# open-speech/HTK

Hardware: AMD Instinct MI355X
Metric: herest_gmm_frame_state_loglik_per_sec (higher is better)
Workload: dtype f32 (scores: bf16x3 split operands, fp32 accumulate) + f64 (alpha / beta with fp32-transcendental log-add, accumulators); 1 GPU; HERest EM iteration (pass + accumulator all-reduce + model update), 5000 tied states x 16 mix, D=39, 1250 x 500-frame utterances per GPU (BASELINE config[2]: 10k utterances sharded 8-way); states=5000, mix=16, utts_per_gpu=1250, frames=500, chunks=1, update=HERest -m 3 -v 0.01, on the device

## Files before the change

### htk_amd/csrc/comm.hip

```cpp
#include <hip/hip_runtime.h>
#include <dlfcn.h>
#include <cstdlib>
#include <cstring>
#include <algorithm>
#include "internal.h"
#include "hipcheck.h"

typedef struct { char internal[128]; } rcclId;
typedef void *rcclComm;
typedef int (*fnGetUniqueId)(rcclId *);
typedef int (*fnCommInitRank)(rcclComm *, int, rcclId, int);
typedef int (*fnAllReduce)(const void *, void *, size_t, int, int, rcclComm, hipStream_t);
typedef int (*fnCommDestroy)(rcclComm);
typedef const char *(*fnGetErrorString)(int);

static struct { void *h; fnGetUniqueId getId; fnCommInitRank init; fnAllReduce allReduce; fnCommDestroy destroy; fnGetErrorString err; } g_rccl;

static int rccl_bind()
{
   if (g_rccl.h) return HTKAMD_OK;
   const char *names[] = {"librccl.so.1", "librccl.so", "/opt/rocm/lib/librccl.so.1", nullptr};
   void *h = nullptr;
   for (int i = 0; names[i] && !h; i++) h = dlopen(names[i], RTLD_NOW | RTLD_GLOBAL);
   if (!h) { htkamd_set_error("comm: RCCL not found (librccl.so.1): %s", dlerror()); return HTKAMD_ENODEV; }
// ... 57 lines not shown
}

__global__ void k_wire_pack(const double *__restrict__ v, float *__restrict__ w, size_t n)
{
   for (size_t i = (size_t)blockIdx.x * blockDim.x + threadIdx.x; i < n; i += (size_t)gridDim.x * blockDim.x) w[i] = (float)v[i];
}
__global__ void k_wire_unpack(const float *__restrict__ w, double *__restrict__ v, size_t n)
{
   for (size_t i = (size_t)blockIdx.x * blockDim.x + threadIdx.x; i < n; i += (size_t)gridDim.x * blockDim.x) v[i] = (double)w[i];
}

extern "C" int htkamd_accs_wire_round(htkamd_accs *a, void *stream)
{
   if (!a) { htkamd_set_error("accs_wire_round: NULL argument"); return HTKAMD_EINVAL; }
   const size_t bulk = a->lay.nEgs;
   float *w = nullptr;
   HIPCHECK(hipMalloc(&w, sizeof(float) * bulk));
   k_wire_pack<<<1024, 256, 0, (hipStream_t)stream>>>(a->d_vec, w, bulk);
   HIPCHECK(hipGetLastError());
   k_wire_unpack<<<1024, 256, 0, (hipStream_t)stream>>>(w, a->d_vec, bulk);
   HIPCHECK(hipGetLastError());
   HIPCHECK(hipStreamSynchronize((hipStream_t)stream));
   HIPCHECK(hipFree(w));
   return HTKAMD_OK;
}

extern "C" int htkamd_accs_allreduce_wire(htkamd_accs *a, htkamd_comm *c, int wire, void *stream)
{
   if (wire == HTKAMD_WIRE_F64) return htkamd_accs_allreduce(a, c, stream);
   if (!a || !c || wire != HTKAMD_WIRE_F32) { htkamd_set_error("accs_allreduce_wire: bad argument"); return HTKAMD_EINVAL; }
   if (c->nRanks == 1) return HTKAMD_OK;
   const size_t bulk = a->lay.nEgs, tail = a->lay.total - bulk;
   if (c->wireCap < bulk) {
      if (c->d_wire) HIPCHECK(hipFree(c->d_wire));
      c->d_wire = nullptr; c->wireCap = 0;
      HIPCHECK(hipMalloc(&c->d_wire, sizeof(float) * bulk));
      c->wireCap = bulk;
   }
   hipStream_t st = (hipStream_t)stream;
   k_wire_pack<<<1024, 256, 0, st>>>(a->d_vec, c->d_wire, bulk);
   HIPCHECK(hipGetLastError());
   RCCLCHECK(g_rccl.allReduce(c->d_wire, c->d_wire, bulk, 7 , 0 , c->c, st));
   RCCLCHECK(g_rccl.allReduce(a->d_vec + bulk, a->d_vec + bulk, tail, 8 , 0, c->c, st));
   k_wire_unpack<<<1024, 256, 0, st>>>(c->d_wire, a->d_vec, bulk);
   HIPCHECK(hipGetLastError());
   return HTKAMD_OK;
}

extern "C" int htkamd_accs_state_ranges(htkamd_accs *a, int state0, int state1, int withRest, size_t off[7], size_t len[7], int *n)
{
   if (!a || !off || !len || !n) { htkamd_set_error("accs_state_ranges: NULL argument"); return HTKAMD_EINVAL; }
   const htkamd_model *m = a->m;
   if (state0 < 0 || state1 > m->S || state0 > state1) { htkamd_set_error("accs_state_ranges: states [%d, %d) outside the set's %d", state0, state1, m->S); return HTKAMD_EINVAL; }
   if (a->stateOrder == 0) {
      a->stateOrder = (m->G == m->C && m->NSt <= 1 && !m->tiedMix) ? 1 : -1;
      for (int c = 0; c < m->C && a->stateOrder == 1; c++) if (m->h_compGauss[c] != c) a->stateOrder = -1;
   }
   if (a->stateOrder < 0) { htkamd_set_error("accs_state_ranges: the set's components do not own their Gaussians in state order (shared pdfs, several streams or tied mixtures): exchange the vector whole"); return HTKAMD_EMODEL; }
   const size_t g0 = (size_t)m->h_stateCompOff[state0], g1 = (size_t)m->h_stateCompOff[state1], D = (size_t)m->D;
   int k = 0;
   auto put = [&](size_t o, size_t l) { if (l) { off[k] = o; len[k] = l; k++; } };
   put(a->lay.mu + g0 * D, (g1 - g0) * D); put(a->lay.muOcc + g0, g1 - g0);
   put(a->lay.va + g0 * D, (g1 - g0) * D); put(a->lay.vaOcc + g0, g1 - g0);
   put(a->lay.wt + g0, g1 - g0); put(a->lay.wtOcc + (size_t)state0, (size_t)(state1 - state0));
   if (withRest) put(a->lay.tr, a->lay.nEgs - a->lay.tr);
   *n = k;
   return HTKAMD_OK;
}

struct RangeSet { size_t off[7], len[7], start[8]; int n; };
template <typename W, bool PACK>
__global__ void k_ranges(double *__restrict__ v, W *__restrict__ w, RangeSet r)
{
   const size_t total = r.start[r.n];
   for (size_t i = (size_t)blockIdx.x * blockDim.x + threadIdx.x; i < total; i += (size_t)gridDim.x * blockDim.x) {
      int k = 0;
      while (k + 1 < r.n && i >= r.start[k + 1]) k++;
      const size_t j = r.off[k] + (i - r.start[k]);
      if (PACK) w[i] = (W)v[j]; else v[j] = (double)w[i];
   }
}

static int ranges_launch(htkamd_accs *a, int n, const size_t *off, const size_t *len, int wire, void *buf, hipStream_t st, bool pack, size_t *totalOut)
{
   if (!a || n < 0 || n > 7 || (n && (!off || !len)) || (wire != HTKAMD_WIRE_F32 && wire != HTKAMD_WIRE_F64)) { htkamd_set_error("accs ranges: bad argument"); return HTKAMD_EINVAL; }
   RangeSet r; r.n = n; r.start[0] = 0;
   for (int k = 0; k < n; k++) {
      if (off[k] + len[k] > a->lay.total) { htkamd_set_error("accs ranges: range %d beyond the vector", k); return HTKAMD_EINVAL; }
      r.off[k] = off[k]; r.len[k] = len[k]; r.start[k + 1] = r.start[k] + len[k];
   }
   if (totalOut) *totalOut = r.start[n];
   if (r.start[n] == 0) return HTKAMD_OK;
   if (!buf) { htkamd_set_error("accs ranges: NULL buffer"); return HTKAMD_EINVAL; }
   const unsigned blocks = (unsigned)std::min<size_t>((r.start[n] + 255) / 256, 2048);
   if (wire == HTKAMD_WIRE_F32) { if (pack) k_ranges<float, true><<<blocks, 256, 0, st>>>(a->d_vec, (float *)buf, r); else k_ranges<float, false><<<blocks, 256, 0, st>>>(a->d_vec, (float *)buf, r); }
   else { if (pack) k_ranges<double, true><<<blocks, 256, 0, st>>>(a->d_vec, (double *)buf, r); else k_ranges<double, false><<<blocks, 256, 0, st>>>(a->d_vec, (double *)buf, r); }
   HIPCHECK(hipGetLastError());
   return HTKAMD_OK;
}

extern "C" int htkamd_accs_pack_ranges(htkamd_accs *a, int n, const size_t *off, const size_t *len, int wire, void *dst, void *stream)
{
   return ranges_launch(a, n, off, len, wire, dst, (hipStream_t)stream, true, nullptr);
}

extern "C" int htkamd_accs_unpack_ranges(htkamd_accs *a, int n, const size_t *off, const size_t *len, int wire, const void *src, void *stream)
{
   return ranges_launch(a, n, off, len, wire, (void *)src, (hipStream_t)stream, false, nullptr);
}

extern "C" int htkamd_accs_allreduce_states(htkamd_accs *a, htkamd_comm *c, int wire, int state0, int state1, int withRest, void *stream)
// ... 42 lines not shown
```

### htk_amd/csrc/fb.hip

```cpp
#include <hip/hip_runtime.h>
#include <cstdio>
#include <cstdlib>
#include <cstring>
#include <cmath>
#include <algorithm>
#include <vector>
#include <thread>
#include <mutex>
#include <condition_variable>
#include <functional>
#include "internal.h"
#include "hipcheck.h"
#include "kernels.h"
#include "devbuf.h"

static constexpr char fbOwner[] = "fb";
typedef DevBufT<fbOwner> DevBuf;

struct PrepPool {
   std::vector<std::thread> th;
   std::mutex mu;
   std::condition_variable cvGo, cvDone;
   std::function<void(int)> job;
   int generation = 0, pending = 0, nJobs = 0;
// ... 83 lines not shown
   {
      for_each([](auto &v, int) { v.clear(); });
      outp = beta = gam = 0; frameStates = 0; nCellsMax = QMax = TMax = 1; nThrMax = 64; rc = HTKAMD_OK; err[0] = 0;
   }
};

struct UttClasses {
   static constexpr int N = 13;
   struct Range { int first, n; };
   static int index(int family, int W) { return W == 0 ? 4 : (family ? 4 * family + 1 : 0) + (W == 1 ? 0 : W == 2 ? 1 : W == 4 ? 2 : 3); }
   void set(const std::vector<int> (&cls)[N], std::vector<int> &list)
   {
      list.clear();
      for (int c = 0; c < N; c++) { list.insert(list.end(), cls[c].begin(), cls[c].end()); off[c + 1] = (int)list.size(); }
   }
   Range of(int family, int W) const { const int c = index(family, W); return {off[c], off[c + 1] - off[c]}; }
   Range general() const { return of(FB_LANE_PER_MODEL, 0); } int nGeneral() const { return general().n; }
   int nLr() const { return off[N] - of(FB_LEFT_TO_RIGHT, 1).first; }
   bool anyOffLr() const { return of(FB_LEFT_TO_RIGHT, 1).first > 0; }
private:
   int off[N + 1] = {};
};

struct ResLayout {
   size_t nUtt;
   size_t status() const { return sizeof(double) * nUtt; }
   size_t counter() const { return (sizeof(double) + sizeof(int)) * nUtt; }
   size_t flag() const { return counter() + sizeof(int); } size_t bytes() const { return counter() + 2 * sizeof(int); }
};

enum { UTT_NO_TEE = 1, UTT_ALL_LR = 2 };

struct htkamd_fb : BatchTables {
   htkamd_model *m = nullptr;
   int nUtt = 0;
   int debug = 0;
   int forceGeneral = 0;
   int noStatePath = 0;
   int noLrPath = 0;
   int topoVersion = 0;
   std::vector<unsigned char> uttFlags;
   UttClasses cls;
   size_t gamTotal = 0, betaWTotal = 0, alphaWTotal = 0;
   int totalFrames = 0, nCellsMax = 1, QMax = 1, TMax = 1, blockDim = 64;
   long long frameStates = 0;
   const float *dX = nullptr;
   DevBuf d_arena;
   DevBuf d_qLo, d_qHi, d_aLo, d_aHi, d_outp, d_beta, d_gam, d_alpha, d_pr;
   DevBuf d_betaW;
   DevBuf d_tmE, d_tmMaxP;
   DevBuf d_outpU;
   DevBuf d_alphaW, d_qBeam, d_aBeam, d_trPart, d_hits, d_hitCtl;
   DevBuf d_sink;
   DevBuf d_stCnt, d_stBucket;
   DevBuf d_laneRec;
   bool mixStateLast = false;
   bool mixDeferred = false;
   FbArgs *faMix = nullptr;
   const int *qBeamLast = nullptr;
   DevBuf d_transOff, d_trOccOff, d_counter;
   DevBuf d_rec, d_recSorted, d_recCtl;
   int recCapForce = 0;
   PrepPool *pool = nullptr; std::vector<PrepChunk> *chunks = nullptr;
   void *h_arena = nullptr; size_t h_arenaCap = 0;
   void *h_res = nullptr; size_t h_resCap = 0;
   hipEvent_t evRes = nullptr; bool resPending = false;
   bool f16Pass = false;
   hipEvent_t ev[6] = {}, evK[2] = {}, evCopy = nullptr;
   hipStream_t resStream = nullptr;
   bool timed = false, copyPending = false, scored = false;
   int evMode = 0, evModeLast = 0;
   ResLayout res() const { return {(size_t)nUtt}; }
};

static bool compat_revisit(const htkamd_model *m) { return (m->compat & HTKAMD_COMPAT_STREAM_REVISIT) && m->NSt > 1 && m->NSt != 3 && !m->tiedMix; }

extern "C" int htkamd_fb_create(htkamd_model *m, htkamd_fb **out)
{
   if (!m || !out) { htkamd_set_error("fb_create: NULL argument"); return HTKAMD_EINVAL; }
   if (m->fullc) { htkamd_set_error("fb_create: forward-backward on FULLC models is not supported yet (its mixture statistics are diagonal)"); return HTKAMD_EMODEL; }
   if (m->maxM > 4096) { htkamd_set_error("fb_create: %d mixture components per state not supported", m->maxM); return HTKAMD_EMODEL; }
   htkamd_fb *fb = new htkamd_fb();
   fb->m = m;
   auto fail = [&](const char *what, hipError_t e) { htkamd_set_error("fb_create: %s: %s", what, hipGetErrorString(e)); htkamd_fb_destroy(fb); return HTKAMD_EHIP; };
   hipError_t e;
   for (hipEvent_t *v : {&fb->ev[0], &fb->ev[1], &fb->ev[2], &fb->ev[3], &fb->ev[4], &fb->ev[5], &fb->evK[0], &fb->evK[1]})
      if ((e = hipEventCreate(v)) != hipSuccess) return fail("hipEventCreate", e);
   if ((e = hipEventCreateWithFlags(&fb->evCopy, hipEventDisableTiming)) != hipSuccess) return fail("hipEventCreate", e);
   if ((e = hipStreamCreateWithFlags(&fb->resStream, hipStreamNonBlocking)) != hipSuccess) return fail("hipStreamCreate", e);
   int rc;
   if ((rc = fb->d_counter.reserve(64)) || (rc = fb->d_transOff.reserve(sizeof(int) * (m->nT + 1))) || (rc = fb->d_trOccOff.reserve(sizeof(int) * (m->nT + 1)))) { htkamd_fb_destroy(fb); return rc; }
   if ((e = hipMemcpy(fb->d_transOff.p, m->h_transOff, sizeof(int) * (m->nT + 1), hipMemcpyHostToDevice)) != hipSuccess ||
       (e = hipMemcpy(fb->d_trOccOff.p, m->h_trOccOff, sizeof(int) * (m->nT + 1), hipMemcpyHostToDevice)) != hipSuccess) return fail("hipMemcpy", e);
   *out = fb;
   return HTKAMD_OK;
}

extern "C" void htkamd_fb_destroy(htkamd_fb *fb)
{
   if (!fb) return;
   if (fb->h_arena) (void)hipHostFree(fb->h_arena);
   if (fb->h_res) (void)hipHostFree(fb->h_res);
   delete fb->pool; delete fb->chunks; delete fb->faMix;
   for (hipEvent_t v : fb->ev) if (v) (void)hipEventDestroy(v);
   for (hipEvent_t v : {fb->evCopy, fb->evRes, fb->evK[0], fb->evK[1]}) if (v) (void)hipEventDestroy(v);
   if (fb->resStream) (void)hipStreamDestroy(fb->resStream);
   delete fb;
// ... 415 lines not shown
   fa.stateCompOff = m->d_stateCompOff; fa.compGauss = m->d_compGauss;
   fa.NSt = m->NSt; fa.outpU = (const float *)fb->d_outpU.p; fa.dimStream = m->d_dimStream;
   fa.compatRevisit = compat_revisit(m) && !fb->nextSame.empty(); fa.nextSame = fb->nextSame.dev;
   fa.transOff = (const int *)fb->d_transOff.p; fa.trOccOff = (const int *)fb->d_trOccOff.p;
   fa.compLogWt = m->d_compLogWt; fa.gparam = m->d_gparam; fa.mean = m->d_mean; fa.laddTab = m->d_laddTab;
   fa.PS = m->PS; fa.D = m->D; fa.maxN = m->maxN; fa.maxM = m->maxM;
   fa.nCellsMax = fb->nCellsMax; fa.QMax = fb->QMax; fa.TMax = fb->TMax;
   fa.acc = accs->d_vec; fa.lay = accs->lay;
   fa.pruneInit = cfg->pruneInit; fa.pruneInc = cfg->pruneInc; fa.pruneLim = cfg->pruneLim;
   fa.minLogExp = m->minLogExp; fa.minFrwdP = cfg->minFrwdP; fa.uFlags = cfg->uFlags;
   fa.gamTotal = fb->gamTotal; fa.gamOffByUtt = fb->gamOff.dev; fa.gamChunkUtt = fb->gamChunkUtt.dev;
   return fa;
}

struct LdsSizes { size_t beta, alpha; };
static LdsSizes fb_lds_sizes(const FbArgs &fa)
{
   const size_t nc = fa.nCellsMax, qm = fa.QMax + 3, mn = fa.maxN, tm = (size_t)fa.TMax + 3;
   auto r8 = [](size_t x) { return (x + 7) & ~(size_t)7; };
   const size_t ldsTab = r8((size_t)LADD_NK * (LADD_DEG + 1) * 8);
   return {2 * r8(nc * 8) + r8(qm * 8) + r8(nc * mn * 4) + 4 * r8(qm * 4) + r8(32) + ldsTab,
           2 * r8(nc * 8) + r8(3 * nc * 8) + r8(qm * 8) + r8(nc * (mn + 1) * 8) + ldsTab + r8(3 * nc * 4) + 2 * r8(nc * mn * 4) + 4 * r8(qm * 4) + 2 * r8(tm * 2)};
}

static const int clsW[4] = {1, 2, 4, 8};

static int fb_reserve_lr(htkamd_fb *fb, const htkamd_fb_config *cfg, FbArgs &fa, bool fastLadd, hipStream_t s)
{
   const htkamd_model *m = fb->m;
   int rc;
   size_t rows = 0;
   for (int W : clsW) rows += (size_t)fb->cls.of(FB_LEFT_TO_RIGHT, W).n * htkamd_stats_lr_chunks(fb->TMax) * W;
   const size_t nfr = fb->totalFrames ? fb->totalFrames : 1;
   if ((rc = fb->d_laneRec.reserve(sizeof(LaneRec) * (fb->slotState.size() + 1))) || (rc = fb->d_sink.reserve(256))) return rc;
   fa.laneRec = (LaneRec *)fb->d_laneRec.p; fa.sink = (double *)fb->d_sink.p;
   if ((rc = fb->d_alphaW.reserve(sizeof(double) * (fb->alphaWTotal + 64))) || (rc = fb->d_qBeam.reserve(sizeof(int) * (nfr + 2))) ||
       (rc = fb->d_aBeam.reserve(sizeof(int) * (nfr + 2))) || (rc = fb->d_trPart.reserve(sizeof(double) * htkamd_stats_lr_row_doubles() * (rows + 256))) ||
       (rc = fb->d_hits.reserve(sizeof(MixHit) * (rows * htkamd_stats_lr_region_cap() + 64))) || (rc = fb->d_hitCtl.reserve(sizeof(int) * (rows + 1))))
      return rc;
   fa.alphaW = (double *)fb->d_alphaW.p; fa.qBeam = (int *)fb->d_qBeam.p; fa.aBeam = (int *)fb->d_aBeam.p; fa.trPart = (double *)fb->d_trPart.p;
   fa.hits = (MixHit *)fb->d_hits.p; fa.hitCtl = (int *)fb->d_hitCtl.p; fa.nHitRegions = (int)rows; fa.hitRegionCap = htkamd_stats_lr_region_cap();
   fa.hitSlots = (m->NSt > 1 || m->tiedMix) ? 1 : 0;
   fa.qBeamNP = fb->qBeamNP.dev;
   if (htkamd_beta_lr_is_lean(fa, fastLadd)) fa.qBeam = const_cast<int *>(fb->qBeamNP.dev);
   fb->qBeamLast = fa.qBeam;
   fb->mixStateLast = false;
   fa.fastMath = fastLadd ? 1 : 0;
   if (fb->recCapForce == 0 && !fa.hitSlots && m->maxM <= 16 && (m->D == 39 || m->D == 26 || m->D == 13) &&
       (cfg->uFlags & (HTKAMD_UPMEANS | HTKAMD_UPVARS | HTKAMD_UPMIXES))) {
      size_t cap = 64;
      while (cap < 65536 && cap * (size_t)m->S < (size_t)16 * fb->totalFrames) cap <<= 1;
      while (cap > 64 && cap * (size_t)m->S * sizeof(HitS) > ((size_t)1 << 30)) cap >>= 1;
      { const char *e = getenv("HTKAMD_ST_CAP"); if (e && atoi(e) > 0) cap = (size_t)atoi(e); }
      if ((rc = fb->d_stCnt.reserve(sizeof(int) * (3 * (size_t)m->S + 4))) || (rc = fb->d_stBucket.reserve(sizeof(HitS) * cap * (size_t)m->S))) return rc;
      fb->mixStateLast = true;
      fa.stCnt = (int *)fb->d_stCnt.p; fa.nTiedStates = m->S; fa.stBucket = (HitS *)fb->d_stBucket.p; fa.stCap = (int)cap;
      HIPCHECK(hipMemsetAsync(fa.stCnt, 0, sizeof(int) * (3 * (size_t)m->S + 4), s));
   }
   return HTKAMD_OK;
}

struct FamilyKernels { int family; int (*beta)(const FbArgs &, int, bool, hipStream_t); int (*alpha)(const FbArgs &, int, bool, hipStream_t); };
static const FamilyKernels familyKernels[] = {{FB_LANE_PER_MODEL, htkamd_launch_beta_w, htkamd_launch_alpha_w},
                                              {FB_LANE_PER_STATE, htkamd_launch_beta_s, htkamd_launch_alpha_s},
                                              {FB_LEFT_TO_RIGHT, htkamd_launch_beta_lr, htkamd_launch_alpha_lr}};

static int fb_recursions(htkamd_fb *fb, const FbArgs &fa, const LdsSizes &lds, bool fastLadd, bool noEv, hipStream_t s)
{
   int rc;
   for (int pass = 0; pass < 2; pass++) {
      FbArgs fc = fa;
      const UttClasses::Range g = fb->cls.general();
      fc.uttList = fb->uttList.dev + g.first; fc.nList = g.n;
      if (g.n > 0 && (rc = pass == 0 ? htkamd_launch_beta(fc, fb->blockDim, lds.beta, s) : htkamd_launch_alpha(fc, fb->blockDim, lds.alpha, s))) return rc;
      for (const FamilyKernels &k : familyKernels)
         for (int c = 3; c >= 0; c--) {
            const UttClasses::Range r = fb->cls.of(k.family, clsW[c]);
            fc.uttList = fb->uttList.dev + r.first; fc.nList = r.n;
            if ((rc = (pass == 0 ? k.beta : k.alpha)(fc, clsW[c], fastLadd, s))) return rc;
         }
      if (!noEv) HIPCHECK(hipEventRecord(fb->ev[2 + pass], s));
   }
   return HTKAMD_OK;
}

static int fb_stats_lr(htkamd_fb *fb, const FbArgs &fa, bool fastLadd, bool noEv, hipStream_t s)
{
   int rc;
   FbArgs fc = fa;
   size_t rowOff = 0;
   for (int c = 3; c >= 0; c--) {
      const UttClasses::Range r = fb->cls.of(FB_LEFT_TO_RIGHT, clsW[c]);
      fc.uttList = fb->uttList.dev + r.first; fc.nList = r.n;
      fc.trPart = fa.trPart ? fa.trPart + rowOff * htkamd_stats_lr_row_doubles() : nullptr;
      fc.hits = fa.hits ? fa.hits + rowOff * htkamd_stats_lr_region_cap() : nullptr; fc.hitCtl = fa.hitCtl ? fa.hitCtl + rowOff : nullptr;
      rowOff += (size_t)fc.nList * htkamd_stats_lr_chunks(fb->TMax) * clsW[c];
      if ((rc = htkamd_launch_stats_lr(fc, clsW[c], fastLadd, s))) return rc;
   }
   if (!noEv) HIPCHECK(hipEventRecord(fb->ev[4], s));
   return HTKAMD_OK;
}

static int fb_mix_stats(htkamd_fb *fb, const htkamd_fb_config *cfg, FbArgs &fa, bool defer, hipStream_t s)
{
   const htkamd_model *m = fb->m;
   const int nLr = fb->cls.nLr();
   int rc;
   if (!(cfg->uFlags & (HTKAMD_UPMEANS | HTKAMD_UPVARS | HTKAMD_UPMIXES))) return HTKAMD_OK;
   if ((cfg->uFlags & (HTKAMD_UPMEANS | HTKAMD_UPVARS)) && fb->recCapForce >= 0) {
      const size_t cap = fb->recCapForce > 0 ? (size_t)fb->recCapForce : std::min<size_t>((size_t)16 * fb->totalFrames + 4096, (size_t)1 << 30);
// ... 297 lines not shown
```

### htk_amd/csrc/fb_kernels.hip

```cpp
#include <hip/hip_runtime.h>
#include <cstring>
#include <cstdlib>
#include "internal.h"
#include "hipcheck.h"
#include "kernels.h"
#include "ladd.h"

#define ladd(x, y, mle) ladd_tab((x), (y), (mle), ltab)

#define EXPFLOOR (-100.0)

struct CellMeta {
   int q, i, N, mc0, ms0;
};

struct LdsCarve {
   char *p;
   __device__ explicit LdsCarve(void *base) : p((char *)base) {}
   template <typename T> __device__ T *take(size_t n)
   {
      T *r = (T *)p;
      p += ((n * sizeof(T) + 7) & ~(size_t)7);
      return r;
   }
// ... 846 lines not shown
   const bool upMu = a.uFlags & HTKAMD_UPMEANS, upVa = a.uFlags & HTKAMD_UPVARS;
   const int nWaves = (gridDim.x * blockDim.x) >> 6;
   for (int g = (blockIdx.x * blockDim.x + threadIdx.x) >> 6; g < G; g += nWaves) {
      const int r0 = start[g], r1 = start[g + 1];
      if (r0 == r1) continue;
      for (int k0 = 0; k0 < D; k0 += 64) {
         const int k = k0 + lane;
         const float mean = (k < D) ? a.mean[(size_t)g * D + k] : 0.0f;
         double sMu = 0.0, sVa = 0.0, sL = 0.0;
         for (int rb = r0; rb < r1; rb += 64) {
            const int nb = (r1 - rb < 64) ? r1 - rb : 64;
            MixRec mine; mine.frame = 0; mine.L = 0.0;
            if (lane < nb) mine = a.recSorted[rb + lane];
            sL += mine.L;
            for (int i = 0; i < nb; i += 4) {
               float xv[4]; double Lv[4];
#pragma unroll
               for (int e = 0; e < 4; e++) {
                  const int ii = (i + e < nb) ? i + e : nb - 1;
                  const int fr = __shfl(mine.frame, ii);
                  Lv[e] = (i + e < nb) ? __shfl(mine.L, ii) : 0.0;
                  xv[e] = (k < D) ? a.X[(size_t)fr * D + k] : 0.0f;
               }
#pragma unroll
               for (int e = 0; e < 4; e++) {
                  if (i + e >= nb) break;
                  const float z = xv[e] - mean;
                  const double L = Lv[e];
                  if (upMu && upVa) {
                     const float zl = (float)((double)z * L);
                     sMu += (double)zl; sVa += (double)(z * zl);
                  } else if (upMu) sMu += (double)z * L;
                  else if (upVa) sVa += (double)(z * z) * L;
               }
            }
         }
         if (k < D) {
            if (upMu && sMu != 0.0) atomicAdd(a.acc + a.lay.mu + (size_t)g * D + k, sMu);
            if (upVa && sVa != 0.0) atomicAdd(a.acc + a.lay.va + (size_t)g * D + k, sVa);
         }
         if (k0 == 0) {
#pragma unroll
            for (int o = 32; o > 0; o >>= 1) sL += __shfl_xor(sL, o);
            if (lane == 0) {
               if (upMu) atomicAdd(a.acc + a.lay.muOcc + g, sL);
               if (upVa) atomicAdd(a.acc + a.lay.vaOcc + g, sL);
            }
         }
      }
   }
}

#define MS_EU 8
template <int DT, int MODE>
__global__ __launch_bounds__(64, MS_EU) void k_mixstate(FbArgs a)
{
#define MS_CHUNK 32
#define MS_CAP 128
#define MS_PARTS 4
   constexpr int GS = 16, HPS = 64 / GS, NQ = (DT + 1) / 2, XS = (DT + 3) & ~3;
   constexpr int CH = MS_CHUNK;
   __shared__ float xs[CH * XS];
   __shared__ double Lt[CH][GS];
   __shared__ double hSeed[CH];
   const int st = a.stBase + blockIdx.x, lane = threadIdx.x, grp = lane / GS, sub = lane % GS;
   const int nst = a.stCnt[st] < a.stCap ? a.stCnt[st] : a.stCap;
   const int part = blockIdx.y;
   const int r0 = part * MS_CAP, r1 = (part == (int)gridDim.y - 1 || r0 + MS_CAP > nst) ? nst : r0 + MS_CAP;
   if (r0 >= nst) return;
   const HitS *bucket = a.stBucket + (size_t)st * a.stCap;
   const int c0 = a.stateCompOff[st], M = a.stateCompOff[st + 1] - c0;
   const bool single = (M == 1 || a.maxM == 1);
   constexpr bool upMu = (MODE & 1) != 0, upVa = (MODE & 2) != 0;
   const bool upWt = a.uFlags & HTKAMD_UPMIXES;
   __shared__ float4 pl[NQ][GS];
   int g = 0;
   float wt = 0.0f, gcst = 0.0f;
   if (sub < M) {
      g = a.compGauss[c0 + sub];
      wt = a.compLogWt[c0 + sub];
      gcst = a.gparam[(size_t)g * a.PS + 2 * DT];
      if (grp == 0) {
         const float4 *P4 = (const float4 *)(a.gparam + (size_t)g * a.PS);
#pragma unroll
         for (int q = 0; q < NQ; q++) { const float4 pv = P4[q]; pl[q][sub] = make_float4(pv.x, pv.z, pv.y, pv.w); }
      }
   }
   float meanR[GS];
   const int gOfLane = (lane < M) ? a.compGauss[c0 + lane] : 0;
#pragma unroll
   for (int m = 0; m < GS; m++) { const int gm_ = __builtin_amdgcn_readlane(gOfLane, m); meanR[m] = (m < M && lane < DT) ? a.mean[(size_t)gm_ * DT + lane] : 0.0f; }
   double sMu[GS], sVa[GS];
#pragma unroll
   for (int m = 0; m < GS; m++) { sMu[m] = 0.0; sVa[m] = 0.0; }
   double wtAcc = 0.0;
   int nTriples = 0;
   const double minF = uniform_f64((double)a.minFrwdP);

   for (int base = r0; base < r1; base += CH) {
      const int n = (r1 - base < CH) ? r1 - base : CH;
      __syncthreads();
      int hfr = 0;
      if (lane < n) { const HitS h = bucket[base + lane]; hfr = h.frame; hSeed[lane] = h.seed; }
      for (int r = 0; r < n; r++) {
         const int fr = __builtin_amdgcn_readlane(hfr, r);
         if (lane < DT)
// ... 25 lines not shown
                  sum += tt[0];
                  if (2 * q + 1 < DT) sum += tt[1];
               }
               const float prob = -0.5f * sum;
               const double x = (seed + (double)wt) + (double)prob;
               if (-x < minF) { pass = true; Lr = a.fastMath ? (double)__builtin_amdgcn_exp2f((float)x * 1.44269504088896341f) : exp(x); }
            }
         }
         if (have) Lt[h][sub] = pass ? Lr : 0.0;
         wtAcc += pass ? Lr : 0.0;
         nTriples += pass ? 1 : 0;
      }
      __syncthreads();
      if (upMu || upVa) {
         unsigned long long bmAll[GS];
#pragma unroll
         for (int m4 = 0; m4 < GS; m4 += 4) {
            double Lq[4];
#pragma unroll
            for (int i = 0; i < 4; i++) Lq[i] = (lane < n) ? Lt[lane][m4 + i] : 0.0;
#pragma unroll
            for (int i = 0; i < 4; i++) bmAll[m4 + i] = __ballot(Lq[i] != 0.0);
         }
#pragma unroll
         for (int m = 0; m < GS; m++) {
            if (m < M) {
               unsigned long long bm = bmAll[m];
               double mu = sMu[m], va = sVa[m];
               const float mean = meanR[m];
               while (bm) {
                  double Lv[4]; float xv[4];
#pragma unroll
                  for (int i = 0; i < 4; i++) {
                     const bool live = bm != 0;
                     const int h = live ? (int)__builtin_ctzll(bm) : 0;
                     bm &= bm - 1;
                     Lv[i] = live ? Lt[h][m] : 0.0;
                     xv[i] = xs[h * XS + (lane < DT ? lane : 0)];
                  }
#pragma unroll
                  for (int i = 0; i < 4; i++) {
                     const double L = Lv[i];
                     const float z = xv[i] - mean;
                     if constexpr (upMu && upVa) { const float zl = (float)((double)z * L); mu += (double)zl; va += (double)(z * zl); }
                     else if constexpr (upMu) mu += (double)z * L;
                     else va += (double)(z * z) * L;
                  }
               }
               sMu[m] = mu; sVa[m] = va;
            }
         }
      }
   }
#pragma unroll
   for (int m = 0; m < GS; m++) {
      if (m < M && lane < DT) {
         const int gm = a.compGauss[c0 + m];
         if (upMu && sMu[m] != 0.0) atomicAdd(a.acc + a.lay.mu + (size_t)gm * DT + lane, sMu[m]);
         if (upVa && sVa[m] != 0.0) atomicAdd(a.acc + a.lay.va + (size_t)gm * DT + lane, sVa[m]);
      }
   }
   double w = wtAcc;
   w += __shfl_xor(w, 16); w += __shfl_xor(w, 32);
   if (grp == 0 && sub < M && w != 0.0) {
      if (upWt) atomicAdd(a.acc + a.lay.wt + c0 + sub, w);
      if (upMu) atomicAdd(a.acc + a.lay.muOcc + g, w);
      if (upVa) atomicAdd(a.acc + a.lay.vaOcc + g, w);
   }
#pragma unroll
   for (int o = 32; o > 0; o >>= 1) nTriples += __shfl_xor(nTriples, o);
   if (lane == 0) { if (part == 0) a.stCnt[a.nTiedStates + 4 + 2 * st] = nst; atomicAdd(a.stCnt + a.nTiedStates + 5 + 2 * st, nTriples); }
   double so = (sub < M) ? w : 0.0;
#pragma unroll
   for (int o = GS / 2; o > 0; o >>= 1) so += __shfl_xor(so, o);
   if (lane == 0 && so != 0.0) atomicAdd(a.acc + a.lay.wtOcc + st, so);
}

bool htkamd_mixstate_applies(const FbArgs &a) { return a.stCnt && a.stBucket && !a.hitSlots && a.maxM <= 16 && (a.D == 39 || a.D == 26 || a.D == 13); }
int htkamd_launch_mixstate_range(const FbArgs &a_in, int st0, int st1, hipStream_t s)
{
   if (st0 < 0 || st1 > a_in.nTiedStates || st0 > st1) { htkamd_set_error("mixture statistics: state range [%d, %d) outside the set's %d", st0, st1, a_in.nTiedStates); return HTKAMD_EINVAL; }
   if (st0 == st1) return HTKAMD_OK;
   FbArgs a = a_in;
   a.stBase = st0;
   const int S = st1 - st0;
   const int mode = ((a.uFlags & HTKAMD_UPMEANS) ? 1 : 0) | ((a.uFlags & HTKAMD_UPVARS) ? 2 : 0);
#define MS_LAUNCH(DT_) \
   do { \
      if (mode == 3) hipLaunchKernelGGL((k_mixstate<DT_, 3>), dim3(S, MS_PARTS), dim3(64), 0, s, a); \
      else if (mode == 1) hipLaunchKernelGGL((k_mixstate<DT_, 1>), dim3(S, MS_PARTS), dim3(64), 0, s, a); \
      else if (mode == 2) hipLaunchKernelGGL((k_mixstate<DT_, 2>), dim3(S, MS_PARTS), dim3(64), 0, s, a); \
      else hipLaunchKernelGGL((k_mixstate<DT_, 0>), dim3(S, MS_PARTS), dim3(64), 0, s, a); \
   } while (0)
   if (a.D == 39) MS_LAUNCH(39); else if (a.D == 26) MS_LAUNCH(26); else MS_LAUNCH(13);
#undef MS_LAUNCH
   HIPCHECK(hipGetLastError());
   return HTKAMD_OK;
}

static int set_lds_limit(const void *fn, size_t lds)
{
   if (lds > 64 * 1024)
      HIPCHECK(hipFuncSetAttribute(fn, hipFuncAttributeMaxDynamicSharedMemorySize, (int)lds));
   return HTKAMD_OK;
}

int htkamd_launch_beta(const FbArgs &a, int blockDim, size_t lds, hipStream_t s)
{
   int rc = set_lds_limit((const void *)k_beta, lds);
   if (rc) return rc;
   hipLaunchKernelGGL(k_beta, dim3(a.nList), dim3(blockDim), lds, s, a);
   HIPCHECK(hipGetLastError());
   return HTKAMD_OK;
}

int htkamd_launch_alpha(const FbArgs &a, int blockDim, size_t lds, hipStream_t s)
{
   int rc = set_lds_limit((const void *)k_alpha, lds);
   if (rc) return rc;
   hipLaunchKernelGGL(k_alpha, dim3(a.nList), dim3(blockDim), lds, s, a);
   HIPCHECK(hipGetLastError());
   return HTKAMD_OK;
}

int htkamd_launch_mixstats(const FbArgs &a_in, hipStream_t s, bool dense, bool listed, bool deferState)
{
   if (!dense && !listed) return HTKAMD_OK;
   FbArgs a = a_in;
   dense = dense && a.gamTotal > 0;
   const bool stateOnly = listed && !dense && htkamd_mixstate_applies(a);
   if (stateOnly) a.rec = nullptr;
// ... 421 lines not shown
```

### htk_amd/csrc/internal.h

```cpp
#ifndef HTKAMD_INTERNAL_H
#define HTKAMD_INTERNAL_H

#include <stddef.h>
#include <stdint.h>
#include <stdio.h>
#include "../../include/htk_amd.h"

#ifdef __cplusplus
extern "C" {
#endif

#define LZERO    (-1.0E10)
#define LSMALL   (-0.5E10)
#define MINEARG  (-708.3)
#define MINLARG  2.45E-308
#define HTK_TPI  6.28318530717959
#define MINMIX   1.0E-5
#define LMINMIX  (-11.5129254649702)

void htkamd_set_error(const char *fmt, ...);

void htkamd_slf_put_word(FILE *f, const char *s);
void htkamd_slf_sort_arcs(int *order, int nArcs, const int *arcStart, const int *arcEnd, const int *nodeRank);

// ... 84 lines not shown
   int vecSize, blockSize;
   int nBias; float *bias;
   float det;
   int mrows, mcols; float *mat;
};

struct htkamd_model {
   int D, S, C, G, nT, H, maxN, maxM;
   int PS;
   int   *h_stateCompOff, *h_compGauss, *h_transN, *h_transOff, *h_hmmTrans, *h_hmmStateOff, *h_hmmState, *h_minDur;
   int   *h_trOccOff;
   unsigned char *h_transLR;
   float *h_mean, *h_var, *h_ivar, *h_gconst, *h_compWeight, *h_compLogWt, *h_transP;
   float *d_gparam;
   double *d_laddTab;
   float *d_mean, *d_ivar, *d_gconst, *d_compLogWt, *d_transP;
   int   *d_stateCompOff, *d_compGauss, *d_transN, *d_transOff;
   float *d_var, *d_compWeight;
   int   *d_trOccOff, *d_hmmTrans, *d_hmmStateOff, *d_hmmState;
   void  *d_updScratch; size_t updScratchCap;
   void  *evUpd; int updPending;
   void  *h_updPin;
   int    topoVersion;
   void  *obRing;
   int    hostStale;
   float *d_mfmaTab;
   int   *d_stateTileOff;
   int   *d_tileState;
   int    mfmaNS, nTiles;
   void  *d_bf16Tab;
   int    bf16NC;
   int    bf16Dense;
   void  *d_f16Tab;
   int    f16Wide;
   float *d_f16Ctl;
   int    tabStale;
   int    compat;
   unsigned char *h_rawLogWt, *d_rawLogWt;
   int    fastUse;
   int   *h_meanLeader, *h_varLeader, *h_varGroupSize;
   int   *d_shareTab;
   int    shareMuMem, shareVaMem;
   int    NSt;
   int   *h_dimStream, *h_gaussStream, *d_dimStream, *d_gaussStream;
   int    tiedMix, tmPool;
   float  tmBeam;
   int   *h_tmPoolOff, *d_tmPoolOff;
   float *h_streamWt, *d_streamWt;
   int   *d_msCompOff;
   int   *h_scanOrder;
   int    fullc, FPS;
   float *h_invCov, *d_fparam;
   double minLogExp;
};

void htkamd_outp_ring_free(void *ring);
int htkamd_model_refresh_mfma_device(struct htkamd_model *m, void *stream);
int htkamd_model_refresh_bf16_device(struct htkamd_model *m, void *stream);
int htkamd_model_refresh_f16_device(struct htkamd_model *m, void *stream);
__attribute__((visibility("hidden"))) int htkamd_model_params_changed(struct htkamd_model *m, void *stream, int fromDevice);
__attribute__((visibility("hidden"))) int htkamd_model_table_current(const struct htkamd_model *m, int path, void *stream);
int htkamd_model_f16_flag(struct htkamd_model *m, void *stream, int *flag);
#define HTKAMD_F16_EMODEL 1
#define HTKAMD_F16_EFEAT  2
int htkamd_model_device_tables(struct htkamd_model *m);
static inline size_t htkamd_tri_size(int D) { return (size_t)D * (D + 1) / 2; }
int htkamd_model_sync_host(struct htkamd_model *m);
void htkamd_model_refresh_topology(struct htkamd_model *m);
int htkamd_update_models(struct htkamd_model *m, const htkamd_accs_layout *lay, const double *acc,
                         const htkamd_update_config *cfg, htkamd_update_stats *st);

struct htkamd_accs {
   struct htkamd_model *m;
   htkamd_accs_layout lay;
   double *d_vec;
   int stateOrder;
};

#ifdef __cplusplus
}
#endif
#endif
```

### htk_amd/csrc/kernels.h

```cpp
#ifndef HTKAMD_KERNELS_H
#define HTKAMD_KERNELS_H
#include <hip/hip_runtime.h>
#include <vector>
#include "internal.h"

#define SCORE_TILE_FRAMES 128
#define B16_TASK_FRAMES 128
#define SCORE_TASK_SLOTS  16
#define SCORE_TASK_SLOTS_WIDE 64
#define SCORE_TASK_SLOTS_EXACT 8

struct ScoreTask {
   int frame0;
   int nFrames;
   int slot0;
   int nSlots;
   int outSlot0;
   int ldo;
   size_t outBase;
};

struct ScoreArgs {
   const ScoreTask *tasks = nullptr;
   int nTasks = 0;
// ... 102 lines not shown
   const short *cQ, *cI;
   const short *thrCell;
   const int *slotState;
   const short *sQ;
   const short *taperLo, *taperHi;
   short *qLo, *qHi, *aLo, *aHi;
   const float *X;
   const float *transP;
   float *outp;
   double *beta, *gam, *alphaDbg;
   double *betaW;
   double *alphaW;
   int *qBeam, *aBeam;
   double *trPart;
   double *pr;
   int *status;
   const int *stateCompOff, *compGauss, *transOff, *trOccOff;
   const float *compLogWt, *gparam, *mean;
   const double *laddTab;
   int PS, D, maxN, maxM;
   int nCellsMax, QMax, TMax;
   double *acc;
   htkamd_accs_layout lay;
   double pruneInit, pruneInc, pruneLim, minLogExp;
   float minFrwdP;
   int uFlags;
   size_t gamTotal;
   const size_t *gamOffByUtt;
   const int *gamChunkUtt;
   MixRec *rec, *recSorted;
   int recCap, G;
   int *recCtl;
   int NSt;
   const float *outpU;
   int compatRevisit;
   const int *nextSame;
   const int *dimStream;
   float *tmE;
   float *tmMaxP;
   const int *tmPoolOff;
   int tmPool, totalFrames;
   const ScoreTask *tmTasks; int tmNTasks; const int *tmSlotState; float *tmOut;
   const float *compWeight, *var;
   int tmCombine;
   const float *streamWt;
   MixHit *hits;
   int hitSlots;
   int *hitCtl;
   int nHitRegions, hitRegionCap;
   LaneRec *laneRec;
   const int *qBeamNP;
   int stBase;
   int *stCnt; int nTiedStates; HitS *stBucket; int stCap;
   int fastMath;
   double *sink;
};

int htkamd_launch_beta(const FbArgs &a, int blockDim, size_t lds, hipStream_t s);
int htkamd_launch_alpha(const FbArgs &a, int blockDim, size_t lds, hipStream_t s);
int htkamd_launch_mixstats(const FbArgs &a, hipStream_t s, bool dense, bool listed, bool deferState = false);
bool htkamd_mixstate_applies(const FbArgs &a);
int htkamd_launch_mixstate_range(const FbArgs &a, int st0, int st1, hipStream_t s);
int htkamd_launch_combine_streams(const FbArgs &a, hipStream_t s);
int htkamd_launch_mixstats_ms(const FbArgs &a, hipStream_t s);
int htkamd_launch_tm_score(const FbArgs &a, hipStream_t s);
int htkamd_launch_mixstats_tm(const FbArgs &a, hipStream_t s);
int htkamd_launch_mixhits_streams(const FbArgs &a, bool tied, hipStream_t s);
int htkamd_tm_score_block(const htkamd_model *m, const ScoreArgs &sa, int nRows, float tmBeam, hipStream_t s);
int htkamd_launch_beta_s(const FbArgs &a, int W, bool fast, hipStream_t s);
int htkamd_launch_alpha_s(const FbArgs &a, int W, bool fast, hipStream_t s);
int htkamd_launch_beta_w(const FbArgs &a, int W, bool fast, hipStream_t s);
int htkamd_launch_beta_lr(const FbArgs &a, int W, bool fast, hipStream_t s);
bool htkamd_beta_lr_is_lean(const FbArgs &a, bool fast);
int htkamd_launch_alpha_lr(const FbArgs &a, int W, bool fast, hipStream_t s);
int htkamd_launch_stats_lr(const FbArgs &a, int W, bool fast, hipStream_t s);
int htkamd_stats_lr_chunks(int TMax);
size_t htkamd_stats_lr_row_doubles(void);
int htkamd_stats_lr_region_cap(void);
int htkamd_launch_alpha_w(const FbArgs &a, int W, bool fast, hipStream_t s);

#endif
```

Measured before the change: 29.48 billion frame-state log-lik/s.

## Replace per-state accumulator atomics with partial slots and last-arriver reduction

In the mixture-state statistics kernel, each wavefront handling part of a tied state used to atomicAdd its mean, variance, weight and occupancy sums straight into the global accumulator. Now, when the set has Gaussians in state order, parts write their partial sums to a per-state slot buffer. A ticket counter elects the last-arriving part, which sums all slots and does plain read-modify-write into the accumulator; single-part states write directly without atomics. This removes global fp64 atomic traffic, at the cost of extra slot memory, a fence and ticket handshake, and reliance on each state being owned by exactly one set of cooperating parts. The state-order check is also moved onto the model so both the kernel setup and the comm code can use it.

Measured after the change: 29.64 billion frame-state log-lik/s (median of 6 runs). Within noise of the previous version (+0.5%).

```diff
diff --git a/htk_amd/csrc/comm.hip b/htk_amd/csrc/comm.hip
--- a/htk_amd/csrc/comm.hip
+++ b/htk_amd/csrc/comm.hip
@@ -133,11 +133,7 @@
    if (!a || !off || !len || !n) { htkamd_set_error("accs_state_ranges: NULL argument"); return HTKAMD_EINVAL; }
    const htkamd_model *m = a->m;
    if (state0 < 0 || state1 > m->S || state0 > state1) { htkamd_set_error("accs_state_ranges: states [%d, %d) outside the set's %d", state0, state1, m->S); return HTKAMD_EINVAL; }
-   if (a->stateOrder == 0) {
-      a->stateOrder = (m->G == m->C && m->NSt <= 1 && !m->tiedMix) ? 1 : -1;
-      for (int c = 0; c < m->C && a->stateOrder == 1; c++) if (m->h_compGauss[c] != c) a->stateOrder = -1;
-   }
-   if (a->stateOrder < 0) { htkamd_set_error("accs_state_ranges: the set's components do not own their Gaussians in state order (shared pdfs, several streams or tied mixtures): exchange the vector whole"); return HTKAMD_EMODEL; }
+   if (!htkamd_model_state_order(a->m)) { htkamd_set_error("accs_state_ranges: the set's components do not own their Gaussians in state order (shared pdfs, several streams or tied mixtures): exchange the vector whole"); return HTKAMD_EMODEL; }
    const size_t g0 = (size_t)m->h_stateCompOff[state0], g1 = (size_t)m->h_stateCompOff[state1], D = (size_t)m->D;
    int k = 0;
    auto put = [&](size_t o, size_t l) { if (l) { off[k] = o; len[k] = l; k++; } };
diff --git a/htk_amd/csrc/fb.hip b/htk_amd/csrc/fb.hip
--- a/htk_amd/csrc/fb.hip
+++ b/htk_amd/csrc/fb.hip
@@ -159,7 +159,7 @@
    DevBuf d_outpU;
    DevBuf d_alphaW, d_qBeam, d_aBeam, d_trPart, d_hits, d_hitCtl;
    DevBuf d_sink;
-   DevBuf d_stCnt, d_stBucket;
+   DevBuf d_stCnt, d_stBucket, d_stPart;
    DevBuf d_laneRec;
    bool mixStateLast = false;
    bool mixDeferred = false;
@@ -681,10 +681,15 @@
       while (cap < 65536 && cap * (size_t)m->S < (size_t)16 * fb->totalFrames) cap <<= 1;
       while (cap > 64 && cap * (size_t)m->S * sizeof(HitS) > ((size_t)1 << 30)) cap >>= 1;
       { const char *e = getenv("HTKAMD_ST_CAP"); if (e && atoi(e) > 0) cap = (size_t)atoi(e); }
-      if ((rc = fb->d_stCnt.reserve(sizeof(int) * (3 * (size_t)m->S + 4))) || (rc = fb->d_stBucket.reserve(sizeof(HitS) * cap * (size_t)m->S))) return rc;
+      if ((rc = fb->d_stCnt.reserve(sizeof(int) * MIXSTATE_STCNT_INTS(m->S))) || (rc = fb->d_stBucket.reserve(sizeof(HitS) * cap * (size_t)m->S))) return rc;
       fb->mixStateLast = true;
       fa.stCnt = (int *)fb->d_stCnt.p; fa.nTiedStates = m->S; fa.stBucket = (HitS *)fb->d_stBucket.p; fa.stCap = (int)cap;
-      HIPCHECK(hipMemsetAsync(fa.stCnt, 0, sizeof(int) * (3 * (size_t)m->S + 4), s));
+      HIPCHECK(hipMemsetAsync(fa.stCnt, 0, sizeof(int) * MIXSTATE_STCNT_INTS(m->S), s));
+      const size_t partBytes = sizeof(double) * htkamd_mixstate_part_doubles(m->D, m->S);
+      if (htkamd_model_state_order(fb->m) && partBytes <= ((size_t)1 << 30)) {
+         if ((rc = fb->d_stPart.reserve(partBytes))) return rc;
+         fa.stPart = (double *)fb->d_stPart.p;
+      }
    }
    return HTKAMD_OK;
 }
diff --git a/htk_amd/csrc/fb_kernels.hip b/htk_amd/csrc/fb_kernels.hip
--- a/htk_amd/csrc/fb_kernels.hip
+++ b/htk_amd/csrc/fb_kernels.hip
@@ -922,6 +922,7 @@
 }
 
 #define MS_EU 8
+#define MS_SLOT_DOUBLES(D_) (2 * 16 * (D_) + 16 + 2)
 template <int DT, int MODE>
 __global__ __launch_bounds__(64, MS_EU) void k_mixstate(FbArgs a)
 {
@@ -1053,31 +1054,121 @@
          }
       }
    }
-#pragma unroll
-   for (int m = 0; m < GS; m++) {
-      if (m < M && lane < DT) {
-         const int gm = a.compGauss[c0 + m];
-         if (upMu && sMu[m] != 0.0) atomicAdd(a.acc + a.lay.mu + (size_t)gm * DT + lane, sMu[m]);
-         if (upVa && sVa[m] != 0.0) atomicAdd(a.acc + a.lay.va + (size_t)gm * DT + lane, sVa[m]);
-      }
-   }
    double w = wtAcc;
    w += __shfl_xor(w, 16); w += __shfl_xor(w, 32);
+#pragma unroll
+   for (int o = 32; o > 0; o >>= 1) nTriples += __shfl_xor(nTriples, o);
+   double so = (sub < M) ? w : 0.0;
+#pragma unroll
+   for (int o = GS / 2; o > 0; o >>= 1) so += __shfl_xor(so, o);
+   if (lane == 0 && part == 0) a.stCnt[a.nTiedStates + 4 + 2 * st] = nst;
+   const int nParts = (nst + MS_CAP - 1) / MS_CAP;
+   if (!a.stPart || nParts > MS_PARTS) {
+#pragma unroll
+      for (int m = 0; m < GS; m++) {
+         if (m < M && lane < DT) {
+            const int gm = a.compGauss[c0 + m];
+            if (upMu && sMu[m] != 0.0) atomicAdd(a.acc + a.lay.mu + (size_t)gm * DT + lane, sMu[m]);
+            if (upVa && sVa[m] != 0.0) atomicAdd(a.acc + a.lay.va + (size_t)gm * DT + lane, sVa[m]);
+         }
+      }
+      if (grp == 0 && sub < M && w != 0.0) {
+         if (upWt) atomicAdd(a.acc + a.lay.wt + c0 + sub, w);
+         if (upMu) atomicAdd(a.acc + a.lay.muOcc + g, w);
+         if (upVa) atomicAdd(a.acc + a.lay.vaOcc + g, w);
+      }
+      if (lane == 0) atomicAdd(a.stCnt + a.nTiedStates + 5 + 2 * st, nTriples);
+      if (lane == 0 && so != 0.0) atomicAdd(a.acc + a.lay.wtOcc + st, so);
+      return;
+   }
+   constexpr int SLOT = MS_SLOT_DOUBLES(DT), oVa = GS * DT, oW = 2 * GS * DT, oSo = oW + GS, oNt = oSo + 1;
+   auto add_rows = [&](int m4, const auto &tMu, const auto &tVa) {
+      constexpr int NG = sizeof(tMu) / sizeof(double);
+      double oMu[NG], oVar[NG];
+#pragma unroll
+      for (int i = 0; i < NG; i++) {
+         const bool on = m4 + i < M && lane < DT;
+         oMu[i] = (upMu && on) ? a.acc[a.lay.mu + (size_t)(c0 + m4 + i) * DT + lane] : 0.0;
+         oVar[i] = (upVa && on) ? a.acc[a.lay.va + (size_t)(c0 + m4 + i) * DT + lane] : 0.0;
+      }
+#pragma unroll
+      for (int i = 0; i < NG; i++) {
+         const bool on = m4 + i < M && lane < DT;
+         if (upMu && on && tMu[i] != 0.0) a.acc[a.lay.mu + (size_t)(c0 + m4 + i) * DT + lane] = oMu[i] + tMu[i];
+         if (upVa && on && tVa[i] != 0.0) a.acc[a.lay.va + (size_t)(c0 + m4 + i) * DT + lane] = oVar[i] + tVa[i];
+      }
+   };
+   if (nParts > 1) {
+      double *slots = a.stPart + (size_t)st * MS_PARTS * SLOT, *mine = slots + (size_t)part * SLOT;
+#pragma unroll
+      for (int m = 0; m < GS; m++) {
+         if (m < M && lane < DT) {
+            if (upMu) __hip_atomic_store(mine + m * DT + lane, sMu[m], __ATOMIC_RELAXED, __HIP_MEMORY_SCOPE_AGENT);
+            if (upVa) __hip_atomic_store(mine + oVa + m * DT + lane, sVa[m], __ATOMIC_RELAXED, __HIP_MEMORY_SCOPE_AGENT);
+         }
+      }
+      if (grp == 0 && sub < M) __hip_atomic_store(mine + oW + sub, w, __ATOMIC_RELAXED, __HIP_MEMORY_SCOPE_AGENT);
+      if (lane == 0) { __hip_atomic_store(mine + oSo, so, __ATOMIC_RELAXED, __HIP_MEMORY_SCOPE_AGENT); __hip_atomic_store(mine + oNt, (double)nTriples, __ATOMIC_RELAXED, __HIP_MEMORY_SCOPE_AGENT); }
+      asm volatile("s_waitcnt vmcnt(0)" ::: "memory");
+      int ticket = 0;
+      if (lane == 0) ticket = __hip_atomic_fetch_add(a.stCnt + 3 * a.nTiedStates + 4 + st, 1, __ATOMIC_RELAXED, __HIP_MEMORY_SCOPE_AGENT);
+      ticket = __builtin_amdgcn_readfirstlane(ticket);
+      if (ticket != nParts - 1) return;
+      __builtin_amdgcn_fence(__ATOMIC_ACQUIRE, "agent");
+      asm volatile("s_waitcnt vmcnt(0)" ::: "memory");
+#pragma unroll
+      for (int m2 = 0; m2 < GS; m2 += 2) {
+         double vMu[MS_PARTS][2], vVa[MS_PARTS][2], tMu[2], tVa[2];
+#pragma unroll
+         for (int p = 0; p < MS_PARTS; p++)
+#pragma unroll
+            for (int i = 0; i < 2; i++) {
+               const bool on = m2 + i < M && lane < DT && p < nParts;
+               vMu[p][i] = (upMu && on) ? slots[(size_t)p * SLOT + (m2 + i) * DT + lane] : 0.0;
+               vVa[p][i] = (upVa && on) ? slots[(size_t)p * SLOT + oVa + (m2 + i) * DT + lane] : 0.0;
+            }
+#pragma unroll
+         for (int i = 0; i < 2; i++) {
+            tMu[i] = vMu[0][i]; tVa[i] = vVa[0][i];
+#pragma unroll
+            for (int p = 1; p < MS_PARTS; p++) { tMu[i] += vMu[p][i]; tVa[i] += vVa[p][i]; }
+         }
+         add_rows(m2, tMu, tVa);
+      }
+      double vW[MS_PARTS], vSo[MS_PARTS], vNt[MS_PARTS];
+#pragma unroll
+      for (int p = 0; p < MS_PARTS; p++) {
+         const double *sp = slots + (size_t)p * SLOT;
+         vW[p] = (p < nParts && sub < M) ? sp[oW + sub] : 0.0;
+         vSo[p] = (p < nParts) ? sp[oSo] : 0.0; vNt[p] = (p < nParts) ? sp[oNt] : 0.0;
+      }
+      w = vW[0]; so = vSo[0];
+      double nt = vNt[0];
+#pragma unroll
+      for (int p = 1; p < MS_PARTS; p++) { w += vW[p]; so += vSo[p]; nt += vNt[p]; }
+      nTriples = (int)nt;
+   } else {
+#pragma unroll
+      for (int m4 = 0; m4 < GS; m4 += 4) {
+         double tMu[4], tVa[4];
+#pragma unroll
+         for (int i = 0; i < 4; i++) { tMu[i] = sMu[m4 + i]; tVa[i] = sVa[m4 + i]; }
+         add_rows(m4, tMu, tVa);
+      }
+   }
    if (grp == 0 && sub < M && w != 0.0) {
-      if (upWt) atomicAdd(a.acc + a.lay.wt + c0 + sub, w);
-      if (upMu) atomicAdd(a.acc + a.lay.muOcc + g, w);
-      if (upVa) atomicAdd(a.acc + a.lay.vaOcc + g, w);
-   }
-#pragma unroll
-   for (int o = 32; o > 0; o >>= 1) nTriples += __shfl_xor(nTriples, o);
-   if (lane == 0) { if (part == 0) a.stCnt[a.nTiedStates + 4 + 2 * st] = nst; atomicAdd(a.stCnt + a.nTiedStates + 5 + 2 * st, nTriples); }
-   double so = (sub < M) ? w : 0.0;
-#pragma unroll
-   for (int o = GS / 2; o > 0; o >>= 1) so += __shfl_xor(so, o);
-   if (lane == 0 && so != 0.0) atomicAdd(a.acc + a.lay.wtOcc + st, so);
+      if (upWt) a.acc[a.lay.wt + c0 + sub] += w;
+      if (upMu) a.acc[a.lay.muOcc + c0 + sub] += w;
+      if (upVa) a.acc[a.lay.vaOcc + c0 + sub] += w;
+   }
+   if (lane == 0) {
+      a.stCnt[a.nTiedStates + 5 + 2 * st] = nTriples;
+      if (so != 0.0) a.acc[a.lay.wtOcc + st] += so;
+   }
 }
 
 bool htkamd_mixstate_applies(const FbArgs &a) { return a.stCnt && a.stBucket && !a.hitSlots && a.maxM <= 16 && (a.D == 39 || a.D == 26 || a.D == 13); }
+size_t htkamd_mixstate_part_doubles(int D, int S) { return (size_t)S * MS_PARTS * MS_SLOT_DOUBLES(D); }
 int htkamd_launch_mixstate_range(const FbArgs &a_in, int st0, int st1, hipStream_t s)
 {
    if (st0 < 0 || st1 > a_in.nTiedStates || st0 > st1) { htkamd_set_error("mixture statistics: state range [%d, %d) outside the set's %d", st0, st1, a_in.nTiedStates); return HTKAMD_EINVAL; }
diff --git a/htk_amd/csrc/internal.h b/htk_amd/csrc/internal.h
--- a/htk_amd/csrc/internal.h
+++ b/htk_amd/csrc/internal.h
@@ -160,7 +160,18 @@
    int    fullc, FPS;
    float *h_invCov, *d_fparam;
    double minLogExp;
-};
+   int    stateOrder;
+};
+
+static inline int htkamd_model_state_order(struct htkamd_model *m)
+{
+   if (m->stateOrder == 0) {
+      int c, so = (m->G == m->C && m->NSt <= 1 && !m->tiedMix) ? 1 : -1;
+      for (c = 0; c < m->C && so == 1; c++) if (m->h_compGauss[c] != c) so = -1;
+      m->stateOrder = so;
+   }
+   return m->stateOrder > 0;
+}
 
 void htkamd_outp_ring_free(void *ring);
 int htkamd_model_refresh_mfma_device(struct htkamd_model *m, void *stream);
@@ -182,7 +193,6 @@
    struct htkamd_model *m;
    htkamd_accs_layout lay;
    double *d_vec;
-   int stateOrder;
 };
 
 #ifdef __cplusplus
diff --git a/htk_amd/csrc/kernels.h b/htk_amd/csrc/kernels.h
--- a/htk_amd/csrc/kernels.h
+++ b/htk_amd/csrc/kernels.h
@@ -178,6 +178,7 @@
    const int *qBeamNP;
    int stBase;
    int *stCnt; int nTiedStates; HitS *stBucket; int stCap;
+   double *stPart;
    int fastMath;
    double *sink;
 };
@@ -186,6 +187,8 @@
 int htkamd_launch_alpha(const FbArgs &a, int blockDim, size_t lds, hipStream_t s);
 int htkamd_launch_mixstats(const FbArgs &a, hipStream_t s, bool dense, bool listed, bool deferState = false);
 bool htkamd_mixstate_applies(const FbArgs &a);
+size_t htkamd_mixstate_part_doubles(int D, int S);
+#define MIXSTATE_STCNT_INTS(S) (((4 * (size_t)(S) + 4) + 3) & ~(size_t)3)
 int htkamd_launch_mixstate_range(const FbArgs &a, int st0, int st1, hipStream_t s);
 int htkamd_launch_combine_streams(const FbArgs &a, hipStream_t s);
 int htkamd_launch_mixstats_ms(const FbArgs &a, hipStream_t s);
```
